# thangktran/HardwareAwareOptimalQuantumCircuitCuttingAndKnitting

Hardware: AMD Instinct MI355X
Metric: subcircuit-instances/s (full-knit wall time = ms_per_step), syc 32 p=2 (higher is better)
Workload: dtype f64

## Files before the change

hardwareawareoptimalquantumcircuitcuttingandknitting_amd/_lib.py:

```python
from __future__ import annotations

import ctypes
import os
import threading

_HERE = os.path.dirname(os.path.abspath(__file__))
LIB_PATH = os.environ.get("QKNIT_LIB") or os.path.join(_HERE, "libqknit.so")

c_i32, c_i64, c_u32, c_u64 = ctypes.c_int32, ctypes.c_int64, ctypes.c_uint32, ctypes.c_uint64
c_vp, c_dp, c_lp = ctypes.c_void_p, ctypes.POINTER(ctypes.c_double), ctypes.POINTER(ctypes.c_int64)


class QkPass(ctypes.Structure):
    _fields_ = [("tile_mask", c_u64), ("group_begin", c_i32), ("group_end", c_i32),
                ("flags", c_i32), ("traced_local", c_u32)]


class QkProgram(ctypes.Structure):
    _fields_ = [("n", c_i32), ("n_eff", c_i32), ("m", c_i32), ("n_slots", c_i32),
                ("packed", c_i32), ("n_passes", c_i32), ("passes", ctypes.POINTER(QkPass)),
                ("ops", c_vp), ("groups", c_vp), ("mats", c_vp)]


class QkLowrankPlan(ctypes.Structure):
# ... 41 lines not shown
    "qk_reduce_labels": (c_i32, [c_vp, c_i64, c_vp, c_i64, c_vp, c_vp]),
    "qk_gemm_keyed": (c_i32, [c_vp, c_i64, c_i64, c_i64, c_vp, c_i64, c_vp, c_i64, c_vp, c_i64,
                              c_vp, c_i64, c_vp, ctypes.c_int]),
    "qk_gemm_keyed_pred": (c_i32, [c_vp, c_i64, c_i64, c_i64, c_vp, c_i64, c_vp, c_i64, c_vp, c_i64,
                                   c_vp, c_i64, c_vp, ctypes.c_int, c_vp]),
    "qk_gemm_outer_paired": (c_i32, [c_vp, c_i64, c_i64, c_i64, c_vp, c_i64, c_vp, c_i64, c_vp, c_i64,
                                     c_vp, c_vp]),
    "qk_knit_outer_stream": (c_i32, [c_vp, ctypes.c_int, c_i64, c_vp, c_i64, c_vp, c_i64, ctypes.c_uint64,
                                     ctypes.c_uint64, c_vp]),
    "qk_knit_outer_stream_kind": (c_i32, [ctypes.c_int, c_i64, c_u64, c_u64, c_i64, c_i64,
                                          ctypes.POINTER(ctypes.c_int), ctypes.POINTER(ctypes.c_int)]),
    "qk_knit_outer_stream_range": (c_i32, [c_vp, ctypes.c_int, c_i64, c_vp, c_i64, c_vp, c_i64, ctypes.c_uint64,
                                           ctypes.c_uint64, c_i64, c_i64, c_vp, c_vp]),
    "qk_rank_factors": (c_i32, [c_vp, c_i64, c_vp, c_vp, ctypes.c_double, ctypes.c_double, ctypes.c_double,
                                ctypes.c_int, c_vp, c_vp, c_vp]),
    "qk_prep_workspace_bytes": (c_i32, [c_vp, c_i64, c_i64, ctypes.POINTER(c_i64)]),
    "qk_prep_operands": (c_i32, [c_vp, ctypes.c_int, ctypes.c_int, c_vp, c_vp, c_i64, c_i64, c_vp, ctypes.c_int,
                                 c_vp, c_vp, c_i64, c_i64, c_vp, c_vp, c_vp, c_vp, c_vp, c_vp, c_i64]),
    "qk_compress_operands": (c_i32, [c_vp, ctypes.c_int, ctypes.c_int, c_vp, c_vp, c_i64, c_vp, c_vp, c_vp, c_i64,
                                     c_vp]),
    "qk_compress_operands_ld": (c_i32, [c_vp, ctypes.c_int, ctypes.c_int, c_vp, c_vp, c_i64, c_i64, c_vp, c_i64, c_vp,
                                        c_vp, c_i64, c_i64, c_vp, c_i64]),
    "qk_compress_probe_v": (c_i32, [c_vp, ctypes.c_int, ctypes.c_int, c_vp, c_vp, c_i64, c_i64, c_vp, c_i64, c_vp, c_vp,
                                    c_i64, c_i64, c_vp, c_i64, c_vp, c_i64, c_vp, c_i64]),
    "qk_probe_errors_vpart": (c_i32, [c_vp, ctypes.c_int, ctypes.c_int, c_vp, c_i64, c_i64, c_vp, c_i64, c_vp, c_vp,
                                      c_i64, c_vp, c_vp, ctypes.c_double, ctypes.c_double, c_vp, c_vp, c_vp, c_i64,
                                      c_vp]),
    "qk_probe_workspace_bytes": (c_i32, [c_vp, c_i64, ctypes.POINTER(c_i64)]),
    "qk_probe_errors": (c_i32, [c_vp, ctypes.c_int, ctypes.c_int, c_vp, c_i64, c_i64, c_vp, c_i64, c_vp, c_vp, c_i64,
                                c_i64, c_vp, c_i64, c_vp, c_vp, ctypes.c_double, ctypes.c_double, c_vp, c_vp, c_vp,
# ... 91 lines not shown
```

hardwareawareoptimalquantumcircuitcuttingandknitting_amd/csrc/qknit_plan.hip:

```cpp
#include <hip/hip_runtime.h>

#include <algorithm>
#include <cstdlib>
#include <string>
#include <vector>

#include "internal.h"

namespace {

int pfail(qk_ctx* ctx, int code, const std::string& msg) {
    if (ctx) ctx->err = msg;
    return code;
}

__global__ void qk_pdep_keys_kernel(int64_t n, uint64_t mask, int64_t* keys) {
    for (int64_t x = blockIdx.x * (int64_t)blockDim.x + threadIdx.x; x < n; x += (int64_t)gridDim.x * blockDim.x) {
        uint64_t m = mask, k = 0, bit = 1;
        for (; m; m &= m - 1, bit <<= 1)
            if ((uint64_t)x & bit) k |= m & (~m + 1);
        keys[x] = (int64_t)k;
    }
}

// ... 156 lines not shown
    }
    rc = qk_gemm_keyed(ctx, M, width(fb), K, A, M, X(fb), width(fb), kA, sA, keys(fb), keys(fb) ? 0 : stride_of(fb),
                       out, 0);
    if (!rc && hipGetLastError() != hipSuccess) rc = pfail(ctx, QK_EHIP, "qk_knit: launch failed");
    return rc;
}

}

namespace {

constexpr int LR_RMAX = 8;
constexpr int LR_PROBES = 16;

struct LowrankLayout {
    int64_t xa, xb, g, u, prep, ta, tb, r, a2, b2, e2, k, err, probe, ka, kb, total;
    int64_t prep_bytes, probe_bytes;
};

int lowrank_layout(qk_ctx* ctx, const qk_lowrank_plan* p, LowrankLayout& L, std::string& why) {
    if (!p || p->terms < 2 || p->terms > 64 || (p->terms & 1) || p->rows_a < 1 || p->rows_b < 1 || !p->wt_a ||
        !p->wt_b || !p->probes || p->nbits < 2 || p->nbits > 32) {
        why = "qk_knit_lowrank: need even 2 <= terms <= 64, swept rows, transforms, probes, 2 <= nbits <= 32";
        return QK_EARG;
    }
    if (p->rows_a > INT32_MAX || p->rows_b > INT32_MAX) {
        why = "qk_knit_lowrank: rows_a and rows_b must be at most INT32_MAX";
        return QK_EARG;
    }
    const uint64_t full = (uint64_t(1) << p->nbits) - 1;
    if ((p->mask_a & p->mask_b) || (p->mask_a | p->mask_b) != full || !(p->mask_b & 1)) {
// ... 19 lines not shown
    L.xb = take(K * NB * 8);
    L.g = take(2 * K * K * 8);
    L.u = take(K * LR_PROBES * 8);
    L.prep = take(prep);
    L.ta = take(LR_RMAX * K * 8);
    L.tb = take(LR_RMAX * K * 8);
    L.r = take(8);
    L.a2 = take(LR_RMAX * NA * 8);
    L.b2 = take(LR_RMAX * NB * 8);
    L.e2 = take(2 * LR_PROBES * 8);
    L.k = take(8);
    L.err = take(8);
    L.probe = take(probe);
    L.ka = contiguous_bits(p->mask_a) ? -1 : take(NA * 8);
    L.kb = contiguous_bits(p->mask_b) ? -1 : take(NB * 8);
    L.total = off;
    L.prep_bytes = prep;
    L.probe_bytes = probe;
    return QK_OK;
}

__global__ void qk_copy_i32_kernel(const int32_t* src, int32_t* dst) { *dst = *src; }

}

extern "C" {

int qk_knit_lowrank_workspace_bytes(qk_ctx* ctx, const qk_lowrank_plan* plan, int64_t* bytes) {
    if (!ctx || !bytes) return QK_EARG;
    LowrankLayout L;
// ... 11 lines not shown
    std::string why;
    int rc = lowrank_layout(ctx, p, L, why);
    if (rc) return pfail(ctx, rc, why);
    if (!q_a || !q_b || !out || !workspace || workspace_bytes < L.total)
        return pfail(ctx, QK_EARG, "qk_knit_lowrank: null rows / output, or workspace below qk_knit_lowrank_workspace_bytes");
    if (hipSetDevice(ctx->device) != hipSuccess) return pfail(ctx, QK_EHIP, "qk_knit_lowrank: hipSetDevice");
    char* ws = static_cast<char*>(workspace);
    auto D = [&](int64_t off) { return reinterpret_cast<double*>(ws + off); };
    const int K = p->terms;
    const int64_t NA = int64_t(1) << __builtin_popcountll(p->mask_a), NB = int64_t(1) << __builtin_popcountll(p->mask_b);
    double *XA = D(L.xa), *XB = D(L.xb), *G = D(L.g), *U = D(L.u);
    int32_t* r = reinterpret_cast<int32_t*>(ws + L.r);
    int32_t* k = reinterpret_cast<int32_t*>(ws + L.k);
    rc = qk_prep_operands(ctx, K, (int)p->rows_a, p->wt_a, q_a, NA, NA, XA, (int)p->rows_b, p->wt_b, q_b, NB, NB, XB,
                          p->probes, G, G + K * K, U, D(L.prep), L.prep_bytes);
    if (!rc) rc = qk_rank_factors(ctx, K, G, G + K * K, p->lam_tol, p->s_tol, p->s_abs, LR_RMAX, D(L.ta), D(L.tb), r);
    if (!rc) rc = qk_compress_operands(ctx, K, LR_RMAX, D(L.ta), XA, NA, D(L.a2), D(L.tb), XB, NB, D(L.b2));
    if (!rc)
        rc = qk_probe_errors(ctx, K, LR_RMAX, XA, NA, NA, D(L.a2), NA, U, D(L.b2), NB, NB, p->probes, NB, D(L.e2), r,
                             p->rank_tol, p->rank_tol_rel, k, D(L.err), D(L.probe), L.probe_bytes);
    if (!rc)
        rc = qk_knit_outer_stream_range(ctx, p->nbits, LR_RMAX, D(L.a2), NA, D(L.b2), NB, p->mask_a, p->mask_b, 0,
                                        int64_t(1) << p->nbits, k, out);
    if (rc) return rc;
    int64_t* ka = L.ka >= 0 ? reinterpret_cast<int64_t*>(ws + L.ka) : nullptr;
    int64_t* kb = L.kb >= 0 ? reinterpret_cast<int64_t*>(ws + L.kb) : nullptr;
    if (ka) hipLaunchKernelGGL(qk_pdep_keys_kernel, dim3(grid_of(NA)), dim3(256), 0, ctx->stream, NA, p->mask_a, ka);
    if (kb) hipLaunchKernelGGL(qk_pdep_keys_kernel, dim3(grid_of(NB)), dim3(256), 0, ctx->stream, NB, p->mask_b, kb);
    const int64_t sa = ka ? 0 : int64_t(1) << __builtin_ctzll(p->mask_a);
    const int64_t sb = kb ? 0 : int64_t(1) << __builtin_ctzll(p->mask_b);
    rc = qk_gemm_keyed_pred(ctx, NA, NB, K, XA, NA, XB, NB, ka, sa, kb, sb, out, 0, k);
    if (rc) return rc;
    if (rank_out) hipLaunchKernelGGL(qk_copy_i32_kernel, dim3(1), dim3(1), 0, ctx->stream, k, rank_out);
    if (hipGetLastError() != hipSuccess) return pfail(ctx, QK_EHIP, "qk_knit_lowrank: launch failed");
    return QK_OK;
// ... 4 lines not shown
```

hardwareawareoptimalquantumcircuitcuttingandknitting_amd/csrc/qknit_prep.hip:

```cpp
#include <hip/hip_runtime.h>

#include <cstdint>
#include <string>

#include "internal.h"

namespace {

typedef double d4_t __attribute__((ext_vector_type(4)));
typedef double d2_t __attribute__((ext_vector_type(2)));

constexpr int PK = 64;
constexpr int PCT = 128;
constexpr int PNP = 16;
constexpr int PTH = 512;
constexpr int XLD = PCT + 2;
constexpr int PG_BLK = 10;
constexpr int PPG = PG_BLK * 256;
constexpr int PPA = PPG;
constexpr int PPB = PPG + PK * PNP;
__host__ __device__ constexpr int prep_tri(int bi, int bj) { return bi * 4 - bi * (bi - 1) / 2 + (bj - bi); }

struct PrepSide {
    const double* Wt;
// ... 668 lines not shown
        const double err = sqrt(m);
        const double bound = fmax(tol, rel_tol * sqrt(f));
        const int r = *r_dev;
        if (err_out) *err_out = err;
        const int k = (r > 0 && err <= bound) ? r : 0;
        *k_out = k;
        if (tally) {
            tally[0] += r == 0 ? 1 : 0;
            tally[1] += (r > 0 && k == 0) ? 1 : 0;
            tally[2] = k;
            tally[3] += 1;
        }
    }
}

int probe_grid_d(qk_ctx* ctx, int64_t NA) {
    const int64_t blocks = (NA + 63) / 64;
    const int64_t cap = (int64_t)(ctx->cus > 0 ? ctx->cus : 256) * 2;
    return (int)(blocks < cap ? (blocks > 0 ? blocks : 1) : cap);
}

int fail(qk_ctx* ctx, int code, const char* msg) {
    ctx->err = msg;
    return code;
}

#ifndef QK_PREP_SPLIT
#define QK_PREP_SPLIT 1
#endif
bool prep_split(qk_ctx* ctx, int64_t NA, int64_t NB) {
// ... 125 lines not shown
    const int gd = probe_grid_d(ctx, NA);
    if (work_bytes < (int64_t)(PV_GRID * PV_PART + gd * PE) * (int64_t)sizeof(double))
        return fail(ctx, QK_EARG, "qk_probe_errors_vpart: workspace too small (qk_probe_workspace_bytes)");
    if (hipSetDevice(ctx->device) != hipSuccess) return fail(ctx, QK_EHIP, "qk_probe_errors_vpart: hipSetDevice");
    double* epart = work + PV_GRID * PV_PART;
    hipLaunchKernelGGL(qk_probe_d_kernel, dim3(gd), dim3(256), 0, ctx->stream, K, rmax, XA, ldx, NA, A2, lda2, U, vpart,
                       (int)gv, epart);
    hipLaunchKernelGGL(qk_probe_accept_kernel, dim3(1), dim3(256), 0, ctx->stream, epart, gd, r_dev, tol, rel_tol, e2,
                       k_out, err_out, tally);
    const hipError_t e = hipGetLastError();
    if (e != hipSuccess)
        return fail(ctx, QK_EHIP, (std::string("qk_probe_errors_vpart: ") + hipGetErrorString(e)).c_str());
    return QK_OK;
}

int qk_probe_workspace_bytes(qk_ctx* ctx, int64_t NA, int64_t* bytes) {
    if (!ctx || !bytes) return QK_EARG;
    *bytes = (int64_t)(PV_GRID * PV_PART + probe_grid_d(ctx, NA) * PE) * (int64_t)sizeof(double);
    return QK_OK;
}

int qk_probe_errors(qk_ctx* ctx, int K, int rmax, const double* XA, int64_t ldx, int64_t NA, const double* A2,
                    int64_t lda2, const double* U, const double* B2, int64_t ldb2, int64_t NB, const double* probes,
                    int64_t ldp, double* e2, const int32_t* r_dev, double tol, double rel_tol, int32_t* k_out,
                    double* err_out, double* work, int64_t work_bytes) {
    return qk_probe_errors_tally(ctx, K, rmax, XA, ldx, NA, A2, lda2, U, B2, ldb2, NB, probes, ldp, e2, r_dev, tol,
                                 rel_tol, k_out, err_out, work, work_bytes, nullptr);
}

int qk_probe_errors_tally(qk_ctx* ctx, int K, int rmax, const double* XA, int64_t ldx, int64_t NA, const double* A2,
// ... 62 lines not shown
```

hardwareawareoptimalquantumcircuitcuttingandknitting_amd/csrc/qknit_rank.hip:

```cpp
#include <hip/hip_runtime.h>

#include <cmath>

#include "internal.h"

namespace {

constexpr int RK_K = 64;
constexpr int RK_RC = 32;
constexpr int RK_R = 8;
constexpr int RK_THREADS = 128;

#ifdef QK_RANK_DEBUG
__device__ long long qk_rank_dbg[8];
#define RK_STAMP(i) \
    if (threadIdx.x == 0) qk_rank_dbg[i] = wall_clock64();
#else
#define RK_STAMP(i)
#endif

struct RankArgs {
    int K, rmax;
    const double* GA;
    const double* GB;
    double lam_tol, s_tol, s_abs;
    double* TA;
    double* TB;
    int32_t* r_out;
};

template <int CTRL>
__device__ __forceinline__ double dppd(double v) {
    int2 w = *reinterpret_cast<int2*>(&v);
    w.x = __builtin_amdgcn_mov_dpp(w.x, CTRL, 0xF, 0xF, false);
    w.y = __builtin_amdgcn_mov_dpp(w.y, CTRL, 0xF, 0xF, false);
    return *reinterpret_cast<double*>(&w);
}
template <int CTRL>
__device__ __forceinline__ int dppi(int v) {
    return __builtin_amdgcn_mov_dpp(v, CTRL, 0xF, 0xF, false);
}
__device__ __forceinline__ double readlane_d(double v, int l) {
    int2 w = *reinterpret_cast<int2*>(&v);
// ... 49 lines not shown
        }
    }
    v = bv;
    idx = bi;
}

__global__ __launch_bounds__(RK_THREADS) void qk_rank_factors_kernel(RankArgs a) {
    __shared__ double G[2][RK_K][RK_K + 1];
    __shared__ double L[2][RK_K][RK_RC + 1];
    __shared__ double C[RK_RC][RK_RC + 1];
    __shared__ double Xs[RK_RC][RK_R + 2];
    __shared__ double Ys[RK_RC][RK_R + 2];
    __shared__ double Y[2][RK_R][RK_RC];
    __shared__ int piv[2][RK_RC], nsteps[2], conv[2], rank_s, chol_live[2][2];
    __shared__ double Ts[2][RK_R][RK_K];

    const int tid = threadIdx.x, lane = tid & 63, side = tid >> 6, K = a.K;
    RK_STAMP(0)
    {
        const double* Gs = side ? a.GB : a.GA;
        const int col = lane < K ? lane : K - 1;
        double v[RK_K];
#pragma unroll
        for (int u = 0; u < RK_K; ++u) v[u] = Gs[(u < K ? u : K - 1) * K + col];
#pragma unroll
        for (int u = 0; u < RK_K; ++u)
            if (u < K && lane < K) G[side][u][lane] = v[u];
        __syncthreads();
        RK_STAMP(4)
    }

    double d = lane < K ? G[side][lane][lane] : 0.0;
    bool alive = lane < K;
    double dmax = d;
    {
        int di = lane;
        wargmax(dmax, di);
    }
    bool active = dmax > 0.0, converged = !(dmax > 0.0);
    int steps = 0;
    for (int j = 0; j <= RK_RC; ++j) {
        if (active) {
// ... 100 lines not shown
        const int rx = sd ? rb : ra;
        double* y = Y[sd][t];
        for (int i = rx - 1; i >= 0; --i) {
            double v = sd ? Ys[i][t] : Xs[i][t];
            for (int k = i + 1; k < rx; ++k) v -= L[sd][piv[sd][k]][i] * y[k];
            y[i] = v / L[sd][piv[sd][i]][i];
        }
        for (int i = 0; i < rx; ++i) Ts[sd][t][piv[sd][i]] = y[i];
    }
    __syncthreads();
    for (int e = tid; e < a.rmax * K; e += RK_THREADS) {
        a.TA[e] = Ts[0][e / K][e % K];
        a.TB[e] = Ts[1][e / K][e % K];
    }
    if (tid == 0) *a.r_out = r;
    RK_STAMP(3)
#ifdef QK_RANK_DEBUG
    if (tid == 0) {
        qk_rank_dbg[6] = ra;
        qk_rank_dbg[7] = rb;
    }
#endif
}

}

#ifdef QK_RANK_DEBUG
extern "C" int qk_rank_debug(long long* out) {
    return hipMemcpyFromSymbol(out, HIP_SYMBOL(qk_rank_dbg), sizeof(long long) * 8) == hipSuccess ? 0 : 1;
}
#endif

extern "C" int qk_rank_factors(qk_ctx* ctx, int64_t K, const double* GA, const double* GB, double lam_tol,
                               double s_tol, double s_abs, int rmax, double* TA, double* TB, int32_t* r_out) {
    if (!ctx) return QK_EARG;
    if (K < 1 || K > RK_K || rmax < 1 || rmax > RK_R) {
        ctx->err = "qk_rank_factors: need 1 <= K <= 64 and 1 <= rmax <= 8";
        return QK_EARG;
    }
    if (!GA || !GB || !TA || !TB || !r_out) {
        ctx->err = "qk_rank_factors: null buffer";
        return QK_EARG;
    }
    if (hipSetDevice(ctx->device) != hipSuccess) {
        ctx->err = "qk_rank_factors: hipSetDevice";
        return QK_EHIP;
    }
    RankArgs args{(int)K, rmax, GA, GB, lam_tol, s_tol, s_abs, TA, TB, r_out};
    hipLaunchKernelGGL(qk_rank_factors_kernel, dim3(1), dim3(RK_THREADS), 0, ctx->stream, args);
    const hipError_t e = hipGetLastError();
    if (e != hipSuccess) {
        ctx->err = std::string("qk_rank_factors: ") + hipGetErrorString(e);
        return QK_EHIP;
    }
    return QK_OK;
}
```

hardwareawareoptimalquantumcircuitcuttingandknitting_amd/data_rank.py:

```python
from __future__ import annotations

import numpy as np

LAM_TOL = 1e-12
S_TOL = 1e-13
S_ABS = 1e-15
RC_MAX = 32
R_MAX = 8
K_MAX = 64


def pivoted_cholesky(G: np.ndarray, lam_tol: float = LAM_TOL, rc_max: int = RC_MAX):
    K = G.shape[0]
    d = np.diag(G).astype(np.float64).copy()
    dmax = float(d.max()) if K else 0.0
    if dmax <= 0:
        return np.zeros((K, 0)), [], True
    L = np.zeros((K, rc_max))
    alive = np.ones(K, dtype=bool)
    piv: list = []
    for j in range(rc_max + 1):
        if float(np.maximum(d[alive], 0.0).sum()) <= lam_tol * dmax:
            return L[:, :j], piv, True
        if j == rc_max:
# ... 46 lines not shown
                 s_abs: float = S_ABS, rmax: int = R_MAX, rc_max: int = RC_MAX):
    K = GA.shape[0]
    GA = 0.5 * (GA + GA.T)
    GB = 0.5 * (GB + GB.T)
    LA, pa, oka = pivoted_cholesky(GA, lam_tol, rc_max)
    LB, pb, okb = pivoted_cholesky(GB, lam_tol, rc_max)
    if not (oka and okb) or not pa or not pb:
        return None
    X, Y = cross_factors(LA.T @ LB, s_tol, s_abs, rmax)
    r = X.shape[1]
    if r == 0 or r > rmax:
        return None
    return _side_factor(LA, pa, X, K), _side_factor(LB, pb, Y, K)


data_rank_factors = rank_factors
```

hardwareawareoptimalquantumcircuitcuttingandknitting_amd/engine.py:

```python
from __future__ import annotations

import atexit
import contextlib
import ctypes
import dataclasses
import hashlib
import logging
import os
import threading
from dataclasses import dataclass, field
from time import perf_counter

import numpy as np

from . import _lib
from .fragment_program import (FragmentProgram, JobTable, basis_reduce, build_jobs, compile_fragment,
                               dedup_labels)
from .knit_plan import LabelSpace, deposit_keys, factor_vgate
from .sweep_plan import K_SLOT, EncodedProgram, encode

_torch = None


def torch():
# ... 1371 lines not shown
    from . import data_rank as dr

    T = torch()
    K = GA.shape[0]
    assert GA.shape == (K, K) and GB.shape == (K, K) and GA.is_contiguous() and GB.is_contiguous()
    if out is None:
        out = (T.empty((rmax, K), dtype=T.float64, device=GA.device), T.empty((rmax, K), dtype=T.float64,
                                                                              device=GA.device),
               T.empty(1, dtype=T.int32, device=GA.device))
    TA, TB, r = out
    ctx.check(ctx.lib.qk_rank_factors(ctx.handle, K, GA.data_ptr(), GB.data_ptr(), dr.LAM_TOL, dr.S_TOL, dr.S_ABS,
                                      rmax, TA.data_ptr(), TB.data_ptr(), r.data_ptr()), "qk_rank_factors")
    return TA, TB, r


PREP_COLS = 128
N_PROBES = 16
_PREP_WORK: dict = {}


def prep_ok(K: int, NA: int, NB: int) -> bool:
    return 2 <= K <= 64 and K % 2 == 0 and NA >= PREP_COLS and NB >= PREP_COLS and NA % PREP_COLS == 0 and NB % PREP_COLS == 0


POISON_UNUSED = os.environ.get("QKNIT_POISON_UNUSED", "0") == "1"


def prep_operands(ctx: Context, WtA, qA, WtB, qB, probes, out=None):
    T = torch()
    RA, K = WtA.shape
# ... 69 lines not shown
        A2.fill_(float("nan"))
    gv = -(-NB // CV_COLS)
    vpart = T.empty((gv, 8, N_PROBES), dtype=T.float64, device=XA.device)
    ctx.check(ctx.lib.qk_compress_probe_v(ctx.handle, K, rmax, TA.data_ptr(), src, n, XA.stride(0),
                                          A2.data_ptr() + 8 * base, NA, TB.data_ptr(), XB.data_ptr(), NB, NB,
                                          B2.data_ptr(), NB, probes.data_ptr(), NB, vpart.data_ptr(), vpart.numel()),
              "qk_compress_probe_v")
    return A2, B2, vpart


def compress_probe_v_ok(XA, XB, a_cols=None) -> bool:
    n = XA.shape[1] if a_cols is None else a_cols[1]
    base = 0 if a_cols is None or XA.shape[1] == n else a_cols[0]
    return (n % 2 == 0 and XB.shape[1] % 2 == 0 and XA.stride(0) % 2 == 0 and base % 2 == 0
            and (XA.data_ptr() + 8 * base) % 16 == 0 and XB.data_ptr() % 16 == 0)


_PROBE_WORK: dict = {}
def probe_errors(ctx: Context, XA, A2, U, B2, probes, r=None, tol: float = 0.0, a2_cols: tuple | None = None,
                 rel_tol: float = 0.0, tally=None, vpart=None):
    T = torch()
    K, NA = XA.shape
    rmax = A2.shape[0]
    NB = B2.shape[1]
    assert U.shape == (K, N_PROBES) and probes.shape == (N_PROBES, NB) and B2.shape[0] == rmax
    assert all(t.is_contiguous() for t in (A2, U, B2, probes))
    assert XA.stride(1) == 1 and XA.stride(0) >= NA
    off = 0 if a2_cols is None else a2_cols[0]
    assert (a2_cols is None and A2.shape[1] == NA) or (a2_cols is not None and a2_cols[1] == NA)
    dev = XA.device
# ... 421 lines not shown
```

hardwareawareoptimalquantumcircuitcuttingandknitting_amd/pipeline.py:

```python
from __future__ import annotations

import ctypes
import os
import threading
from dataclasses import dataclass
from time import perf_counter

import numpy as np

from . import _lib, engine
from .fragment_program import JobTable


_PROBES: dict = {}
_PROBES_LOCK = threading.Lock()


def _mm_nt(X, Y):
    L = X.shape[1]
    nb = L // 256 if L % 256 == 0 else 1
    if nb <= 1:
        return X @ Y.T
    Xb = X.view(X.shape[0], nb, 256).transpose(0, 1)
    Yb = Y.reshape(Y.shape[0], nb, 256).transpose(0, 1)
# ... 170 lines not shown
    def device_width(self, fs) -> int:
        return 1 << fs.prog.m

    def fuses_labels(self, fs) -> bool:
        return False

    def bind(self):
        """Follow the caller's current stream (nothing to do on a host backend)."""

    def outer_stream_kernel(self, K, clbits_a, clbits_b, nbits, o_begin=0, o_count=None) -> str:
        return type(self).__name__

    def compress_v(self, TA, XA, TB, XB, probes, a_cols=None, a_width=None):
        return None

    def rank_tally(self, r, k, acc):
        T = engine.torch()
        rv, kv = int(r.reshape(-1)[0]), int(k.reshape(-1)[0])
        acc += T.tensor([int(rv == 0), int(rv > 0 and kv == 0), 0, 1], dtype=T.int64)
        acc[2] = kv


class HipBackend(Backend):

    routes = frozenset(Backend.ROUTES)

    def __init__(self, device: int = 0):
        self.T = engine.torch()
        self.device = device
        self.dev = self.T.device("cuda", device)
# ... 104 lines not shown
        return engine.rank_factors_device(self.ctx, GA, GB)

    def prep_operands(self, WtA, qA, WtB, qB, probes):
        return engine.prep_operands(self.ctx, WtA, qA, WtB, qB, probes)

    fuses_tally = True

    def probe_errors(self, XA, A2, U, B2, probes, r=None, tol=0.0, a2_cols=None, rel_tol=0.0, tally=None, vpart=None):
        return engine.probe_errors(self.ctx, XA, A2, U, B2, probes, r=r, tol=tol, a2_cols=a2_cols, rel_tol=rel_tol,
                                   tally=tally, vpart=vpart)

    def compress_v(self, TA, XA, TB, XB, probes, a_cols=None, a_width=None):
        if os.environ.get("QKNIT_COMPRESS_V", "1") == "0" or not engine.compress_probe_v_ok(XA, XB, a_cols):
            return None
        return engine.compress_probe_v(self.ctx, TA, XA, TB, XB, probes, a_cols=a_cols, a_width=a_width)

    def probe_accept(self, e2, r, tol, rel_tol=0.0):
        return engine.probe_accept(self.ctx, e2, r, tol, rel_tol)

    def rank_tally(self, r, k, acc):
        self.ctx.check(self.ctx.lib.qk_rank_tally(self.ctx.handle, r.data_ptr(), k.data_ptr(), acc.data_ptr()),
                       "qk_rank_tally")

    def compress(self, TA, XA, TB, XB, a_cols=None, a_width=None):
        return engine.compress_operands(self.ctx, TA, XA, TB, XB, a_cols=a_cols, a_width=a_width)

    def knit_select(self, A, B, clbits_a, clbits_b, nbits, accuracy, k_dev=None):
        return engine.knit_select(self.ctx, A, B, clbits_a, clbits_b, nbits, accuracy, k_dev=k_dev)

    def npd_pairs(self, keys, vals):
# ... 567 lines not shown
        if reduce_err is not None:
            e2 = reduce_err(e2)
        n = e2.numel() // 2
        err = e2[:n].max().sqrt()
        bound = T.clamp(self.rank_tol_rel * e2[n:].max().sqrt(), min=self.rank_tol)
        k_eff = T.where((err <= bound) & (r > 0), r, T.zeros_like(r))
        if note:
            self._note_rank(r, k_eff)
        return k_eff, err

    def _prep_dev_rank(self, qs) -> PreparedStep:
        ia, ib = self.order[0], self.order[-1]
        if self._fused_prep(qs):
            x = self._probes(qs[ib].shape[1], qs[ib].device)
            mats, G, U = self._prep_fused(qs, x)
            TA, TB, r = self.be.rank_factors(G[0], G[1])
            return self._compress_and_check(TA, TB, r, mats, U, x)
        mats = self.operands(qs)
        self.last_prep = "torch"
        A, B = mats[ia], mats[ib]
        G = self.T.stack([_mm_nt(A, A), _mm_nt(B, B)])
        TA, TB, r = self.be.rank_factors(G[0].contiguous(), G[1].contiguous())
        A2, B2 = (TA @ A).contiguous(), (TB @ B).contiguous()
        k_eff, _ = self._accept(A, B, A2, B2, self._probes(B.shape[1], B.device), r)
        return PreparedStep(A2, B2, k_eff, mats)

    def _compress_and_check(self, TA, TB, r, mats, U, x) -> PreparedStep:
        ia, ib = self.order[0], self.order[-1]
        a_cols = self._replicated_a_cols()
        kw = {"a_cols": a_cols} if a_cols is not None else {}
        cv = self.be.compress_v(TA, mats[ia], TB, mats[ib], x, **kw)
        check = {}
        if cv is not None:
            A2, B2, check["vpart"] = cv
        else:
            A2, B2 = self.be.compress(TA, mats[ia], TB, mats[ib], **kw)
        XA = mats[ia]
        if a_cols is not None:
            XA = XA[:, a_cols[0]:a_cols[0] + a_cols[1]]
            check["a2_cols"] = a_cols
        tally = self.be.fuses_tally
        if tally:
            check["tally"] = self._tally_for(r.device)
        _, k_eff, _ = self.be.probe_errors(XA, A2, U, B2, x, r=r, tol=self.rank_tol, rel_tol=self.rank_tol_rel,
                                           **check)
# ... 698 lines not shown
```

include/qknit.h:

```cpp
#ifndef QKNIT_H
#define QKNIT_H

#include <stdint.h>

#ifdef __cplusplus
extern "C" {
#endif

#define QK_OK 0
#define QK_EARG 1
#define QK_EHIP 2
#define QK_ESTATE 3

#define QK_TILE_BITS 12
#define QK_FIBER_BITS 4

enum { QK_U1 = 0, QK_D1 = 1, QK_SLOT = 2, QK_U2 = 3, QK_D2 = 4, QK_CX = 5, QK_SWAP = 6, QK_SCALE = 7,
       QK_U1R = 8, QK_U1X = 9, QK_D1R = 10, QK_D2R = 11, QK_SCALER = 12 };

typedef struct qk_op {
    int32_t kind;
    int32_t a, b;
    int32_t e1, e2;
    int32_t slot;
// ... 143 lines not shown

#define QK_COMM_ID_BYTES 128
typedef struct qk_comm qk_comm;
int qk_comm_unique_id(uint8_t* id);
int qk_comm_init(qk_ctx* ctx, const uint8_t* id, int nranks, int rank, qk_comm** out);
int qk_comm_destroy(qk_comm* comm);
int qk_comm_size(qk_comm* comm, int* nranks, int* rank);
int qk_allreduce(qk_ctx* ctx, qk_comm* comm, const double* send, double* recv, int64_t count);
int qk_reduce(qk_ctx* ctx, qk_comm* comm, const double* send, double* recv, int64_t count, int root);
int qk_allgather(qk_ctx* ctx, qk_comm* comm, const double* send, double* recv, int64_t count);
int qk_alltoall(qk_ctx* ctx, qk_comm* comm, const double* send, double* recv, int64_t count);

int qk_rank_factors(qk_ctx* ctx, int64_t K, const double* GA, const double* GB, double lam_tol, double s_tol,
                    double s_abs, int rmax, double* TA, double* TB, int32_t* r_out);

int qk_prep_workspace_bytes(qk_ctx* ctx, int64_t NA, int64_t NB, int64_t* bytes);
int qk_prep_operands(qk_ctx* ctx, int K, int RA, const double* WtA, const double* qA, int64_t ldqA, int64_t NA,
                     double* XA, int RB, const double* WtB, const double* qB, int64_t ldqB, int64_t NB, double* XB,
                     const double* probes, double* GA, double* GB, double* U, double* work, int64_t work_bytes);

int qk_compress_operands(qk_ctx* ctx, int K, int rmax, const double* TA, const double* XA, int64_t NA, double* A2,
                         const double* TB, const double* XB, int64_t NB, double* B2);
int qk_compress_operands_ld(qk_ctx* ctx, int K, int rmax, const double* TA, const double* XA, int64_t NA, int64_t ldxa,
                            double* A2, int64_t lda2, const double* TB, const double* XB, int64_t NB, int64_t ldxb,
                            double* B2, int64_t ldb2);

int qk_compress_probe_v(qk_ctx* ctx, int K, int rmax, const double* TA, const double* XA, int64_t NA, int64_t ldxa,
                        double* A2, int64_t lda2, const double* TB, const double* XB, int64_t NB, int64_t ldxb,
                        double* B2, int64_t ldb2, const double* probes, int64_t ldp, double* vpart,
                        int64_t vpart_doubles);

int qk_probe_errors_vpart(qk_ctx* ctx, int K, int rmax, const double* XA, int64_t ldx, int64_t NA, const double* A2,
                          int64_t lda2, const double* U, const double* vpart, int64_t gv, double* e2,
                          const int32_t* r_dev, double tol, double rel_tol, int32_t* k_out, double* err_out,
                          double* work, int64_t work_bytes, int64_t* tally);

int qk_probe_workspace_bytes(qk_ctx* ctx, int64_t NA, int64_t* bytes);
int qk_probe_errors(qk_ctx* ctx, int K, int rmax, const double* XA, int64_t ldx, int64_t NA, const double* A2,
                    int64_t lda2, const double* U, const double* B2, int64_t ldb2, int64_t NB, const double* probes,
                    int64_t ldp, double* e2, const int32_t* r_dev, double tol, double rel_tol, int32_t* k_out,
                    double* err_out, double* work, int64_t work_bytes);
int qk_probe_errors_tally(qk_ctx* ctx, int K, int rmax, const double* XA, int64_t ldx, int64_t NA, const double* A2,
                          int64_t lda2, const double* U, const double* B2, int64_t ldb2, int64_t NB,
                          const double* probes, int64_t ldp, double* e2, const int32_t* r_dev, double tol,
                          double rel_tol, int32_t* k_out, double* err_out, double* work, int64_t work_bytes,
                          int64_t* tally);
int qk_probe_accept(qk_ctx* ctx, const double* e2, int n, const int32_t* r_dev, double tol, double rel_tol,
                    int32_t* k_out, double* err_out);
int qk_rank_tally(qk_ctx* ctx, const int32_t* r_dev, const int32_t* k_dev, int64_t* acc);

// ... 132 lines not shown
```

Before: 522,500.

## Compute probe V in rank kernel and compress using only pivot columns

The rank-factor kernel now also emits the sorted pivot column lists for each side and computes V = TB·U over the B-side pivots. A new compress kernel multiplies only the pivot rows of X, since the factors are nonzero only on pivot columns. The error check then reuses the precomputed V instead of a separate V-partial reduction. The aim is fewer FMAs and memory reads in compression and a shorter kernel chain, at the cost of more work in the single-block rank kernel and an assumption that T is zero outside the pivots.

```diff
diff --git a/hardwareawareoptimalquantumcircuitcuttingandknitting_amd/_lib.py b/hardwareawareoptimalquantumcircuitcuttingandknitting_amd/_lib.py
--- a/hardwareawareoptimalquantumcircuitcuttingandknitting_amd/_lib.py
+++ b/hardwareawareoptimalquantumcircuitcuttingandknitting_amd/_lib.py
@@ -79,6 +79,11 @@
                                            ctypes.c_uint64, c_i64, c_i64, c_vp, c_vp]),
     "qk_rank_factors": (c_i32, [c_vp, c_i64, c_vp, c_vp, ctypes.c_double, ctypes.c_double, ctypes.c_double,
                                 ctypes.c_int, c_vp, c_vp, c_vp]),
+    "qk_rank_factors_v": (c_i32, [c_vp, c_i64, c_vp, c_vp, ctypes.c_double, ctypes.c_double, ctypes.c_double,
+                                  ctypes.c_int, c_vp, c_vp, c_vp, c_vp, c_vp, c_vp]),
+    "qk_compress_check": (c_i32, [c_vp, ctypes.c_int, ctypes.c_int, c_vp, c_vp, c_vp, c_vp, c_i64, c_i64, c_vp, c_i64,
+                                  c_vp, c_vp, c_i64, c_i64, c_vp, c_i64, c_vp, c_vp, c_vp, ctypes.c_double,
+                                  ctypes.c_double, c_vp, c_vp, c_vp, c_i64, c_vp]),
     "qk_prep_workspace_bytes": (c_i32, [c_vp, c_i64, c_i64, ctypes.POINTER(c_i64)]),
     "qk_prep_operands": (c_i32, [c_vp, ctypes.c_int, ctypes.c_int, c_vp, c_vp, c_i64, c_i64, c_vp, ctypes.c_int,
                                  c_vp, c_vp, c_i64, c_i64, c_vp, c_vp, c_vp, c_vp, c_vp, c_vp, c_i64]),
diff --git a/hardwareawareoptimalquantumcircuitcuttingandknitting_amd/csrc/qknit_plan.hip b/hardwareawareoptimalquantumcircuitcuttingandknitting_amd/csrc/qknit_plan.hip
--- a/hardwareawareoptimalquantumcircuitcuttingandknitting_amd/csrc/qknit_plan.hip
+++ b/hardwareawareoptimalquantumcircuitcuttingandknitting_amd/csrc/qknit_plan.hip
@@ -194,7 +194,7 @@
 constexpr int LR_PROBES = 16;
 
 struct LowrankLayout {
-    int64_t xa, xb, g, u, prep, ta, tb, r, a2, b2, e2, k, err, probe, ka, kb, total;
+    int64_t xa, xb, g, u, prep, ta, tb, r, a2, b2, e2, k, err, probe, ka, kb, v, piv, total;
     int64_t prep_bytes, probe_bytes;
 };
 
@@ -244,6 +244,8 @@
     L.probe = take(probe);
     L.ka = contiguous_bits(p->mask_a) ? -1 : take(NA * 8);
     L.kb = contiguous_bits(p->mask_b) ? -1 : take(NB * 8);
+    L.v = take(LR_RMAX * LR_PROBES * 8);
+    L.piv = take(2 * 33 * 4);
     L.total = off;
     L.prep_bytes = prep;
     L.probe_bytes = probe;
@@ -285,11 +287,23 @@
     int32_t* k = reinterpret_cast<int32_t*>(ws + L.k);
     rc = qk_prep_operands(ctx, K, (int)p->rows_a, p->wt_a, q_a, NA, NA, XA, (int)p->rows_b, p->wt_b, q_b, NB, NB, XB,
                           p->probes, G, G + K * K, U, D(L.prep), L.prep_bytes);
-    if (!rc) rc = qk_rank_factors(ctx, K, G, G + K * K, p->lam_tol, p->s_tol, p->s_abs, LR_RMAX, D(L.ta), D(L.tb), r);
-    if (!rc) rc = qk_compress_operands(ctx, K, LR_RMAX, D(L.ta), XA, NA, D(L.a2), D(L.tb), XB, NB, D(L.b2));
-    if (!rc)
-        rc = qk_probe_errors(ctx, K, LR_RMAX, XA, NA, NA, D(L.a2), NA, U, D(L.b2), NB, NB, p->probes, NB, D(L.e2), r,
-                             p->rank_tol, p->rank_tol_rel, k, D(L.err), D(L.probe), L.probe_bytes);
+    const char* sw = std::getenv("QKNIT_COMPRESS_CHECK");
+    if (!(sw && sw[0] == '0' && !sw[1])) {
+        int32_t* piv = reinterpret_cast<int32_t*>(ws + L.piv);
+        if (!rc)
+            rc = qk_rank_factors_v(ctx, K, G, G + K * K, p->lam_tol, p->s_tol, p->s_abs, LR_RMAX, D(L.ta), D(L.tb), r, U,
+                                   D(L.v), piv);
+        if (!rc)
+            rc = qk_compress_check(ctx, K, LR_RMAX, r, piv, D(L.ta), XA, NA, NA, D(L.a2), NA, D(L.tb), XB, NB, NB,
+                                   D(L.b2), NB, U, D(L.v), D(L.e2), p->rank_tol, p->rank_tol_rel, k, D(L.err), D(L.probe),
+                                   L.probe_bytes, nullptr);
+    } else {
+        if (!rc) rc = qk_rank_factors(ctx, K, G, G + K * K, p->lam_tol, p->s_tol, p->s_abs, LR_RMAX, D(L.ta), D(L.tb), r);
+        if (!rc) rc = qk_compress_operands(ctx, K, LR_RMAX, D(L.ta), XA, NA, D(L.a2), D(L.tb), XB, NB, D(L.b2));
+        if (!rc)
+            rc = qk_probe_errors(ctx, K, LR_RMAX, XA, NA, NA, D(L.a2), NA, U, D(L.b2), NB, NB, p->probes, NB, D(L.e2), r,
+                                 p->rank_tol, p->rank_tol_rel, k, D(L.err), D(L.probe), L.probe_bytes);
+    }
     if (!rc)
         rc = qk_knit_outer_stream_range(ctx, p->nbits, LR_RMAX, D(L.a2), NA, D(L.b2), NB, p->mask_a, p->mask_b, 0,
                                         int64_t(1) << p->nbits, k, out);
diff --git a/hardwareawareoptimalquantumcircuitcuttingandknitting_amd/csrc/qknit_prep.hip b/hardwareawareoptimalquantumcircuitcuttingandknitting_amd/csrc/qknit_prep.hip
--- a/hardwareawareoptimalquantumcircuitcuttingandknitting_amd/csrc/qknit_prep.hip
+++ b/hardwareawareoptimalquantumcircuitcuttingandknitting_amd/csrc/qknit_prep.hip
@@ -706,6 +706,91 @@
     }
 }
 
+constexpr int CC_PIV = 33;
+struct CompressPivArgs {
+    int K, rmax;
+    const int32_t* r_dev;
+    const int32_t* piv;
+    const double* TA;
+    const double* XA;
+    int64_t NA, ldxa;
+    double* A2;
+    int64_t lda2;
+    const double* TB;
+    const double* XB;
+    int64_t NB, ldxb;
+    double* B2;
+    int64_t ldb2;
+    int nA_wg;
+};
+
+__global__ __launch_bounds__(256) void qk_compress_piv_kernel(CompressPivArgs a) {
+    const int tid = threadIdx.x, lane = tid & 63, wave = tid >> 6, K = a.K, rmax = a.rmax;
+    const bool bs = (int)blockIdx.x >= a.nA_wg;
+    const int64_t wg = bs ? (int64_t)blockIdx.x - a.nA_wg : (int64_t)blockIdx.x;
+    const double* Tg = bs ? a.TB : a.TA;
+    const double* X = bs ? a.XB : a.XA;
+    double* out = bs ? a.B2 : a.A2;
+    const int64_t N = bs ? a.NB : a.NA, ld = bs ? a.ldxb : a.ldxa, ldo = bs ? a.ldb2 : a.lda2;
+    const int64_t base = wg * CV_COLS + wave * 128;
+    const int64_t c = base + 2 * lane;
+    const bool valid = c < N;
+    const int64_t cl = valid ? c : N - 2;
+    __shared__ __attribute__((aligned(16))) double Tt[PK][8];
+    __shared__ int pv[CC_PIV];
+    if (*a.r_dev <= 0) return;
+    {
+        double tv[2];
+#pragma unroll
+        for (int i = 0; i < 2; ++i) {
+            const int e = tid + 256 * i, k = e >> 3, j = e & 7;
+            tv[i] = Tg[min(j, rmax - 1) * K + min(k, K - 1)];
+        }
+        const int pe = a.piv[(bs ? CC_PIV : 0) + min(tid, CC_PIV - 1)];
+#pragma unroll
+        for (int i = 0; i < 2; ++i) {
+            const int e = tid + 256 * i, k = e >> 3, j = e & 7;
+            Tt[k][j] = (k < K && j < rmax) ? tv[i] : 0.0;
+        }
+        if (tid < CC_PIV) pv[tid] = pe;
+    }
+    __syncthreads();
+    if (base >= N) return;
+    int np = pv[0];
+    np = np < 0 ? 0 : (np > CC_PIV - 1 ? CC_PIV - 1 : np);
+    d2_t acc[8];
+#pragma unroll
+    for (int j = 0; j < 8; ++j) acc[j] = (d2_t){0.0, 0.0};
+    for (int i0 = 0; i0 < np; i0 += 8) {
+        d2_t xb[8];
+        int kk[8];
+#pragma unroll
+        for (int u = 0; u < 8; ++u) {
+            const int k = i0 + u < np ? pv[1 + i0 + u] : 0;
+            kk[u] = __builtin_amdgcn_readfirstlane(min(max(k, 0), K - 1));
+            xb[u] = *reinterpret_cast<const d2_t*>(X + (int64_t)kk[u] * ld + cl);
+        }
+#pragma unroll
+        for (int u = 0; u < 8; ++u) {
+            const bool on = i0 + u < np;
+#pragma unroll
+            for (int h = 0; h < 4; ++h) {
+                const d2_t tv = *reinterpret_cast<const d2_t*>(&Tt[kk[u]][2 * h]);
+                const double t0 = on ? tv.x : 0.0, t1 = on ? tv.y : 0.0;
+                acc[2 * h].x = fma(t0, xb[u].x, acc[2 * h].x);
+                acc[2 * h].y = fma(t0, xb[u].y, acc[2 * h].y);
+                acc[2 * h + 1].x = fma(t1, xb[u].x, acc[2 * h + 1].x);
+                acc[2 * h + 1].y = fma(t1, xb[u].y, acc[2 * h + 1].y);
+            }
+        }
+    }
+    if (valid) {
+#pragma unroll
+        for (int j = 0; j < 8; ++j)
+            if (j < rmax) *reinterpret_cast<d2_t*>(out + (int64_t)j * ldo + c) = acc[j];
+    }
+}
+
 int probe_grid_d(qk_ctx* ctx, int64_t NA) {
     const int64_t blocks = (NA + 63) / 64;
     const int64_t cap = (int64_t)(ctx->cus > 0 ? ctx->cus : 256) * 2;
@@ -861,6 +946,39 @@
     return QK_OK;
 }
 
+int qk_compress_check(qk_ctx* ctx, int K, int rmax, const int32_t* r_dev, const int32_t* piv, const double* TA,
+                      const double* XA, int64_t NA, int64_t ldxa, double* A2, int64_t lda2, const double* TB,
+                      const double* XB, int64_t NB, int64_t ldxb, double* B2, int64_t ldb2, const double* U,
+                      const double* V, double* e2, double tol, double rel_tol, int32_t* k_out, double* err_out,
+                      double* work, int64_t work_bytes, int64_t* tally) {
+    if (!ctx) return QK_EARG;
+    if (K < 1 || K > PK || rmax < 1 || rmax > 8 || NA < 16 || NA % 16 || NB < 2 || (NB | ldxa | lda2 | ldxb | ldb2) & 1)
+        return fail(ctx, QK_EARG, "qk_compress_check: need 1 <= K <= 64, 1 <= rmax <= 8, NA % 16 == 0, even NB and strides");
+    if (ldxa < NA || lda2 < NA || ldxb < NB || ldb2 < NB)
+        return fail(ctx, QK_EARG, "qk_compress_check: leading dimension below the width");
+    if (!r_dev || !piv || !TA || !XA || !A2 || !TB || !XB || !B2 || !U || !V || !work || (tally && !k_out))
+        return fail(ctx, QK_EARG, "qk_compress_check: null buffer");
+    if ((reinterpret_cast<uintptr_t>(XA) | reinterpret_cast<uintptr_t>(XB) | reinterpret_cast<uintptr_t>(A2) |
+         reinterpret_cast<uintptr_t>(B2)) & 15)
+        return fail(ctx, QK_EARG, "qk_compress_check: operands must be 16-B aligned");
+    const int64_t ga = (NA + CV_COLS - 1) / CV_COLS, gb = (NB + CV_COLS - 1) / CV_COLS;
+    if (ga + gb > INT32_MAX) return fail(ctx, QK_EARG, "qk_compress_check: too many columns");
+    const int gd = probe_grid_d(ctx, NA);
+    if (work_bytes < (int64_t)(PV_GRID * PV_PART + gd * PE) * (int64_t)sizeof(double))
+        return fail(ctx, QK_EARG, "qk_compress_check: workspace too small (qk_probe_workspace_bytes)");
+    if (hipSetDevice(ctx->device) != hipSuccess) return fail(ctx, QK_EHIP, "qk_compress_check: hipSetDevice");
+    CompressPivArgs args{K, rmax, r_dev, piv, TA, XA, NA, ldxa, A2, lda2, TB, XB, NB, ldxb, B2, ldb2, (int)ga};
+    hipLaunchKernelGGL(qk_compress_piv_kernel, dim3((unsigned)(ga + gb)), dim3(256), 0, ctx->stream, args);
+    double* epart = work + PV_GRID * PV_PART;
+    hipLaunchKernelGGL(qk_probe_d_kernel, dim3(gd), dim3(256), 0, ctx->stream, K, rmax, XA, ldxa, NA, A2, lda2, U, V, 1,
+                       epart);
+    hipLaunchKernelGGL(qk_probe_accept_kernel, dim3(1), dim3(256), 0, ctx->stream, epart, gd, r_dev, tol, rel_tol, e2,
+                       k_out, err_out, tally);
+    const hipError_t e = hipGetLastError();
+    if (e != hipSuccess) return fail(ctx, QK_EHIP, (std::string("qk_compress_check: ") + hipGetErrorString(e)).c_str());
+    return QK_OK;
+}
+
 int qk_probe_workspace_bytes(qk_ctx* ctx, int64_t NA, int64_t* bytes) {
     if (!ctx || !bytes) return QK_EARG;
     *bytes = (int64_t)(PV_GRID * PV_PART + probe_grid_d(ctx, NA) * PE) * (int64_t)sizeof(double);
diff --git a/hardwareawareoptimalquantumcircuitcuttingandknitting_amd/csrc/qknit_rank.hip b/hardwareawareoptimalquantumcircuitcuttingandknitting_amd/csrc/qknit_rank.hip
--- a/hardwareawareoptimalquantumcircuitcuttingandknitting_amd/csrc/qknit_rank.hip
+++ b/hardwareawareoptimalquantumcircuitcuttingandknitting_amd/csrc/qknit_rank.hip
@@ -10,6 +10,8 @@
 constexpr int RK_RC = 32;
 constexpr int RK_R = 8;
 constexpr int RK_THREADS = 128;
+constexpr int RK_NP = 16;
+constexpr int RK_PIV = 1 + RK_RC;
 
 #ifdef QK_RANK_DEBUG
 __device__ long long qk_rank_dbg[8];
@@ -27,6 +29,9 @@
     double* TA;
     double* TB;
     int32_t* r_out;
+    const double* U;
+    double* V;
+    int32_t* piv;
 };
 
 template <int CTRL>
@@ -106,6 +111,8 @@
     __shared__ double Y[2][RK_R][RK_RC];
     __shared__ int piv[2][RK_RC], nsteps[2], conv[2], rank_s, chol_live[2][2];
     __shared__ double Ts[2][RK_R][RK_K];
+    __shared__ double Us[RK_K][RK_NP];
+    __shared__ int pivs[2][RK_RC];
 
     const int tid = threadIdx.x, lane = tid & 63, side = tid >> 6, K = a.K;
     RK_STAMP(0)
@@ -115,9 +122,25 @@
         double v[RK_K];
 #pragma unroll
         for (int u = 0; u < RK_K; ++u) v[u] = Gs[(u < K ? u : K - 1) * K + col];
+        constexpr int UPT = RK_K * RK_NP / RK_THREADS;
+        double uv[UPT];
+        if (a.U) {
+#pragma unroll
+            for (int u = 0; u < UPT; ++u) {
+                const int e = tid + RK_THREADS * u;
+                uv[u] = a.U[e < K * RK_NP ? e : K * RK_NP - 1];
+            }
+        }
 #pragma unroll
         for (int u = 0; u < RK_K; ++u)
             if (u < K && lane < K) G[side][u][lane] = v[u];
+        if (a.U) {
+#pragma unroll
+            for (int u = 0; u < UPT; ++u) {
+                const int e = tid + RK_THREADS * u;
+                (&Us[0][0])[e] = e < K * RK_NP ? uv[u] : 0.0;
+            }
+        }
         __syncthreads();
         RK_STAMP(4)
     }
@@ -248,6 +271,24 @@
         a.TB[e] = Ts[1][e / K][e % K];
     }
     if (tid == 0) *a.r_out = r;
+    if (a.U) {
+        const int np = r > 0 ? (side ? rb : ra) : 0;
+        if (lane < np) {
+            const int p = piv[side][lane];
+            int pos = 0;
+            for (int i = 0; i < np; ++i) pos += piv[side][i] < p ? 1 : 0;
+            pivs[side][pos] = p;
+        }
+        __syncthreads();
+        if (lane < RK_PIV) a.piv[side * RK_PIV + lane] = lane == 0 ? np : (lane - 1 < np ? pivs[side][lane - 1] : 0);
+        const int nb = r > 0 ? rb : 0;
+        for (int e = tid; e < RK_R * RK_NP; e += RK_THREADS) {
+            const int j = e / RK_NP, p = e % RK_NP;
+            double s = 0.0;
+            for (int i = 0; i < nb; ++i) s = fma(Ts[1][j][pivs[1][i]], Us[pivs[1][i]][p], s);
+            a.V[e] = j < r ? s : 0.0;
+        }
+    }
     RK_STAMP(3)
 #ifdef QK_RANK_DEBUG
     if (tid == 0) {
@@ -267,12 +308,18 @@
 
 extern "C" int qk_rank_factors(qk_ctx* ctx, int64_t K, const double* GA, const double* GB, double lam_tol,
                                double s_tol, double s_abs, int rmax, double* TA, double* TB, int32_t* r_out) {
+    return qk_rank_factors_v(ctx, K, GA, GB, lam_tol, s_tol, s_abs, rmax, TA, TB, r_out, nullptr, nullptr, nullptr);
+}
+
+extern "C" int qk_rank_factors_v(qk_ctx* ctx, int64_t K, const double* GA, const double* GB, double lam_tol,
+                                 double s_tol, double s_abs, int rmax, double* TA, double* TB, int32_t* r_out,
+                                 const double* U, double* V, int32_t* piv) {
     if (!ctx) return QK_EARG;
     if (K < 1 || K > RK_K || rmax < 1 || rmax > RK_R) {
         ctx->err = "qk_rank_factors: need 1 <= K <= 64 and 1 <= rmax <= 8";
         return QK_EARG;
     }
-    if (!GA || !GB || !TA || !TB || !r_out) {
+    if (!GA || !GB || !TA || !TB || !r_out || (U && (!V || !piv))) {
         ctx->err = "qk_rank_factors: null buffer";
         return QK_EARG;
     }
@@ -280,7 +327,7 @@
         ctx->err = "qk_rank_factors: hipSetDevice";
         return QK_EHIP;
     }
-    RankArgs args{(int)K, rmax, GA, GB, lam_tol, s_tol, s_abs, TA, TB, r_out};
+    RankArgs args{(int)K, rmax, GA, GB, lam_tol, s_tol, s_abs, TA, TB, r_out, U, V, piv};
     hipLaunchKernelGGL(qk_rank_factors_kernel, dim3(1), dim3(RK_THREADS), 0, ctx->stream, args);
     const hipError_t e = hipGetLastError();
     if (e != hipSuccess) {
diff --git a/hardwareawareoptimalquantumcircuitcuttingandknitting_amd/data_rank.py b/hardwareawareoptimalquantumcircuitcuttingandknitting_amd/data_rank.py
--- a/hardwareawareoptimalquantumcircuitcuttingandknitting_amd/data_rank.py
+++ b/hardwareawareoptimalquantumcircuitcuttingandknitting_amd/data_rank.py
@@ -84,4 +84,29 @@
     return _side_factor(LA, pa, X, K), _side_factor(LB, pb, Y, K)
 
 
+def pivot_lists(GA: np.ndarray, GB: np.ndarray, lam_tol: float = LAM_TOL, rc_max: int = RC_MAX) -> np.ndarray:
+    out = np.zeros((2, 1 + rc_max), dtype=np.int32)
+    for s, G in enumerate((GA, GB)):
+        _, piv, _ = pivoted_cholesky(0.5 * (G + G.T), lam_tol, rc_max)
+        out[s, 0] = len(piv)
+        out[s, 1:1 + len(piv)] = sorted(piv)
+    return out
+
+
+def factor_pivots(T: np.ndarray, rc_max: int = RC_MAX) -> np.ndarray:
+    cols = np.flatnonzero(np.any(np.asarray(T) != 0.0, axis=0))
+    assert cols.size <= rc_max
+    out = np.zeros(1 + rc_max, dtype=np.int32)
+    out[0] = cols.size
+    out[1:1 + cols.size] = cols
+    return out
+
+
+def probe_v(TB: np.ndarray, U: np.ndarray, piv: np.ndarray) -> np.ndarray:
+    V = np.zeros((TB.shape[0], U.shape[1]))
+    for b in piv[1:1 + int(piv[0])]:
+        V += np.outer(TB[:, b], U[b])
+    return V
+
+
 data_rank_factors = rank_factors
diff --git a/hardwareawareoptimalquantumcircuitcuttingandknitting_amd/engine.py b/hardwareawareoptimalquantumcircuitcuttingandknitting_amd/engine.py
--- a/hardwareawareoptimalquantumcircuitcuttingandknitting_amd/engine.py
+++ b/hardwareawareoptimalquantumcircuitcuttingandknitting_amd/engine.py
@@ -1409,6 +1409,28 @@
     return TA, TB, r
 
 
+RANK_PIV = 33
+
+
+def rank_factors_v_device(ctx: Context, GA, GB, U, rmax: int = 8):
+    from . import data_rank as dr
+
+    T = torch()
+    K = GA.shape[0]
+    assert GA.shape == (K, K) and GB.shape == (K, K) and GA.is_contiguous() and GB.is_contiguous()
+    assert U.shape == (K, N_PROBES) and U.is_contiguous()
+    dev = GA.device
+    TA = T.empty((rmax, K), dtype=T.float64, device=dev)
+    TB = T.empty((rmax, K), dtype=T.float64, device=dev)
+    ints = T.empty(1 + 2 * RANK_PIV, dtype=T.int32, device=dev)
+    r, piv = ints[:1], ints[1:].view(2, RANK_PIV)
+    V = T.empty((8, N_PROBES), dtype=T.float64, device=dev)
+    ctx.check(ctx.lib.qk_rank_factors_v(ctx.handle, K, GA.data_ptr(), GB.data_ptr(), dr.LAM_TOL, dr.S_TOL, dr.S_ABS,
+                                        rmax, TA.data_ptr(), TB.data_ptr(), r.data_ptr(), U.data_ptr(), V.data_ptr(),
+                                        piv.data_ptr()), "qk_rank_factors_v")
+    return TA, TB, r, piv, V
+
+
 PREP_COLS = 128
 N_PROBES = 16
 _PREP_WORK: dict = {}
@@ -1508,6 +1530,46 @@
     base = 0 if a_cols is None or XA.shape[1] == n else a_cols[0]
     return (n % 2 == 0 and XB.shape[1] % 2 == 0 and XA.stride(0) % 2 == 0 and base % 2 == 0
             and (XA.data_ptr() + 8 * base) % 16 == 0 and XB.data_ptr() % 16 == 0)
+
+
+_CHECK_WORK: dict = {}
+
+
+def compress_check(ctx: Context, TA, XA, TB, XB, U, V, piv, r, tol: float = 0.0, rel_tol: float = 0.0, tally=None,
+                   a_cols: tuple | None = None, a_width: int | None = None):
+    T = torch()
+    rmax, K = TA.shape
+    assert TB.shape == (rmax, K) and XA.shape[0] == K and XB.shape[0] == K
+    assert XA.stride(1) == 1 and XB.is_contiguous() and TA.is_contiguous() and TB.is_contiguous()
+    assert U.shape == (K, N_PROBES) and V.shape == (8, N_PROBES) and U.is_contiguous() and V.is_contiguous()
+    assert piv.dtype == T.int32 and piv.shape == (2, RANK_PIV) and piv.is_contiguous() and r.dtype == T.int32
+    NA = XA.shape[1] if a_width is None else a_width
+    NB = XB.shape[1]
+    dev = XA.device
+    ab = T.empty(rmax * (NA + NB), dtype=T.float64, device=dev)
+    A2 = ab[:rmax * NA].view(rmax, NA)
+    B2 = ab[rmax * NA:].view(rmax, NB)
+    base, n = (0, NA) if a_cols is None else a_cols
+    assert 0 <= base and n >= 16 and n % 16 == 0 and base + n <= NA and XA.shape[1] in (n, NA)
+    src = XA.data_ptr() if XA.shape[1] == n else XA.data_ptr() + 8 * base
+    if a_cols is not None and POISON_UNUSED:
+        A2.fill_(float("nan"))
+    need = ctypes.c_int64()
+    ctx.check(ctx.lib.qk_probe_workspace_bytes(ctx.handle, n, ctypes.byref(need)), "qk_probe_workspace_bytes")
+    key = (str(dev), T.cuda.current_stream(dev).cuda_stream)
+    work = _CHECK_WORK.get(key)
+    if work is None or work.numel() * 8 < need.value:
+        work = _CHECK_WORK[key] = T.empty(max(need.value // 8, 1), dtype=T.float64, device=dev)
+    e2 = T.empty(2 * N_PROBES, dtype=T.float64, device=dev)
+    k = T.empty(1, dtype=T.int32, device=dev)
+    err = T.empty(1, dtype=T.float64, device=dev)
+    assert tally is None or (tally.dtype == T.int64 and tally.numel() == 4)
+    ctx.check(ctx.lib.qk_compress_check(ctx.handle, K, rmax, r.data_ptr(), piv.data_ptr(), TA.data_ptr(), src, n,
+                                        XA.stride(0), A2.data_ptr() + 8 * base, NA, TB.data_ptr(), XB.data_ptr(), NB,
+                                        NB, B2.data_ptr(), NB, U.data_ptr(), V.data_ptr(), e2.data_ptr(), tol, rel_tol,
+                                        k.data_ptr(), err.data_ptr(), work.data_ptr(), work.numel() * 8, _ptr(tally)),
+              "qk_compress_check")
+    return A2, B2, e2, k, err
 
 
 _PROBE_WORK: dict = {}
diff --git a/hardwareawareoptimalquantumcircuitcuttingandknitting_amd/pipeline.py b/hardwareawareoptimalquantumcircuitcuttingandknitting_amd/pipeline.py
--- a/hardwareawareoptimalquantumcircuitcuttingandknitting_amd/pipeline.py
+++ b/hardwareawareoptimalquantumcircuitcuttingandknitting_amd/pipeline.py
@@ -208,6 +208,12 @@
     def compress_v(self, TA, XA, TB, XB, probes, a_cols=None, a_width=None):
         return None
 
+    def rank_factors_v(self, GA, GB, U):
+        return None
+
+    def compress_check(self, TA, XA, TB, XB, U, V, piv, r, tol=0.0, rel_tol=0.0, tally=None, a_cols=None):
+        return None
+
     def rank_tally(self, r, k, acc):
         T = engine.torch()
         rv, kv = int(r.reshape(-1)[0]), int(k.reshape(-1)[0])
@@ -342,6 +348,18 @@
         if os.environ.get("QKNIT_COMPRESS_V", "1") == "0" or not engine.compress_probe_v_ok(XA, XB, a_cols):
             return None
         return engine.compress_probe_v(self.ctx, TA, XA, TB, XB, probes, a_cols=a_cols, a_width=a_width)
+
+    def rank_factors_v(self, GA, GB, U):
+        if os.environ.get("QKNIT_COMPRESS_CHECK", "1") == "0":
+            return None
+        return engine.rank_factors_v_device(self.ctx, GA, GB, U)
+
+    def compress_check(self, TA, XA, TB, XB, U, V, piv, r, tol=0.0, rel_tol=0.0, tally=None, a_cols=None):
+        if not engine.compress_probe_v_ok(XA, XB, a_cols) or (XA.shape[1] if a_cols is None else a_cols[1]) % 16:
+            return None
+        A2, B2, _, k, _ = engine.compress_check(self.ctx, TA, XA, TB, XB, U, V, piv, r, tol=tol, rel_tol=rel_tol,
+                                                tally=tally, a_cols=a_cols)
+        return A2, B2, k
 
     def probe_accept(self, e2, r, tol, rel_tol=0.0):
         return engine.probe_accept(self.ctx, e2, r, tol, rel_tol)
@@ -939,6 +957,9 @@
         if self._fused_prep(qs):
             x = self._probes(qs[ib].shape[1], qs[ib].device)
             mats, G, U = self._prep_fused(qs, x)
+            fv = self.be.rank_factors_v(G[0], G[1], U)
+            if fv is not None:
+                return self._compress_and_check(*fv[:3], mats, U, x, piv=fv[3], V=fv[4])
             TA, TB, r = self.be.rank_factors(G[0], G[1])
             return self._compress_and_check(TA, TB, r, mats, U, x)
         mats = self.operands(qs)
@@ -950,10 +971,21 @@
         k_eff, _ = self._accept(A, B, A2, B2, self._probes(B.shape[1], B.device), r)
         return PreparedStep(A2, B2, k_eff, mats)
 
-    def _compress_and_check(self, TA, TB, r, mats, U, x) -> PreparedStep:
+    def _compress_and_check(self, TA, TB, r, mats, U, x, piv=None, V=None) -> PreparedStep:
         ia, ib = self.order[0], self.order[-1]
         a_cols = self._replicated_a_cols()
         kw = {"a_cols": a_cols} if a_cols is not None else {}
+        if piv is not None:
+            tally = self._tally_for(r.device) if self.be.fuses_tally else None
+            cc = self.be.compress_check(TA, mats[ia], TB, mats[ib], U, V, piv, r, tol=self.rank_tol,
+                                        rel_tol=self.rank_tol_rel, tally=tally, **kw)
+            if cc is not None:
+                A2, B2, k_eff = cc
+                if tally is not None:
+                    self._pending += 1
+                else:
+                    self._note_rank(r, k_eff)
+                return PreparedStep(A2, B2, k_eff, mats)
         cv = self.be.compress_v(TA, mats[ia], TB, mats[ib], x, **kw)
         check = {}
         if cv is not None:
diff --git a/include/qknit.h b/include/qknit.h
--- a/include/qknit.h
+++ b/include/qknit.h
@@ -181,6 +181,10 @@
 int qk_rank_factors(qk_ctx* ctx, int64_t K, const double* GA, const double* GB, double lam_tol, double s_tol,
                     double s_abs, int rmax, double* TA, double* TB, int32_t* r_out);
 
+int qk_rank_factors_v(qk_ctx* ctx, int64_t K, const double* GA, const double* GB, double lam_tol, double s_tol,
+                      double s_abs, int rmax, double* TA, double* TB, int32_t* r_out, const double* U, double* V,
+                      int32_t* piv);
+
 int qk_prep_workspace_bytes(qk_ctx* ctx, int64_t NA, int64_t NB, int64_t* bytes);
 int qk_prep_operands(qk_ctx* ctx, int K, int RA, const double* WtA, const double* qA, int64_t ldqA, int64_t NA,
                      double* XA, int RB, const double* WtB, const double* qB, int64_t ldqB, int64_t NB, double* XB,
@@ -201,6 +205,12 @@
                           int64_t lda2, const double* U, const double* vpart, int64_t gv, double* e2,
                           const int32_t* r_dev, double tol, double rel_tol, int32_t* k_out, double* err_out,
                           double* work, int64_t work_bytes, int64_t* tally);
+
+int qk_compress_check(qk_ctx* ctx, int K, int rmax, const int32_t* r_dev, const int32_t* piv, const double* TA,
+                      const double* XA, int64_t NA, int64_t ldxa, double* A2, int64_t lda2, const double* TB,
+                      const double* XB, int64_t NB, int64_t ldxb, double* B2, int64_t ldb2, const double* U,
+                      const double* V, double* e2, double tol, double rel_tol, int32_t* k_out, double* err_out,
+                      double* work, int64_t work_bytes, int64_t* tally);
 
 int qk_probe_workspace_bytes(qk_ctx* ctx, int64_t NA, int64_t* bytes);
 int qk_probe_errors(qk_ctx* ctx, int K, int rmax, const double* XA, int64_t ldx, int64_t NA, const double* A2,
```

Result: no change. 523,600 (median of 3 runs) (+0.2%).
